# johndpope/SPEAK-hack

Measured on NVIDIA B200. Metric: irfd_train_pairs_per_sec_256, higher is better.
Workload: dtype bf16

## Files before the change

include/irfd_b200.h:

```cpp
#ifndef IRFD_B200_H_
#define IRFD_B200_H_

#include <stddef.h>
#include <stdint.h>

#ifdef __cplusplus
extern "C" {
#endif

#define IRFD_ABI_VERSION 1

#define IRFD_OK 0
#define IRFD_ERR_INVALID_ARGUMENT (-1)
#define IRFD_ERR_CUDA (-2)

typedef struct CUstream_st* irfd_stream_t;

int irfd_abi_version(void);
const char* irfd_last_error(void);

int irfd_conv_gemm_m_tiles(int n, int h, int w);
int irfd_conv_gemm(const void* x, int n, int h, int w, int cin, const void* wk, int cout, int ksize, void* out,
                   void* out2, int mode, const float* bias, const float* nw, const float* noise, const float* sp1,
                   const float* s1, float* stat_sum, float* stat_sq, int force_block_n, irfd_stream_t stream);
// ... 36 lines not shown
                  void* out, long long rows, int c, int relu, int groups, irfd_stream_t stream);
long long irfd_bn_bwd_workspace_bytes(long long rows, int c, int groups);
int irfd_bn_backward(const void* g1, const void* g2, const void* act, const void* z, const float* mean,
                     const float* rstd, const float* gamma, const float* beta, void* dz, void* g_out, float* dgamma,
                     float* dbeta, float grad_beta, int batch_stats, long long rows, int c, int groups, void* workspace,
                     long long workspace_bytes, irfd_stream_t stream);

int irfd_bn_eval_affine_sets(const float* const* running_mean, const float* const* running_var,
                             const float* const* gamma, const float* const* beta, float eps, float* scale, float* shift,
                             int c, int nsets, irfd_stream_t stream);
int irfd_bn_finalize_sets(const float* psum, const float* psq, int tiles, int c, long long count, float eps,
                          float momentum, float* mean, float* rstd, float* const* running_mean,
                          float* const* running_var, int running_updates, int groups, int nsets,
                          irfd_stream_t stream);
int irfd_bn_apply_sets(const void* z, const float* mean, const float* rstd, const float* const* gamma,
                       const float* const* beta, const void* res, const float* mean2, const float* rstd2,
                       const float* const* gamma2, const float* const* beta2, void* out, void* mask_bits,
                       long long rows, int c, int relu, int groups, int nsets, irfd_stream_t stream);
int irfd_bn_backward_sets(const void* g1, const void* g2, const void* act, int act_is_bits, const void* z,
                          const float* mean, const float* rstd, const float* const* gamma, const float* const* beta,
                          void* dz, void* g_out, float* const* dgamma, float* const* dbeta, float grad_beta,
                          int batch_stats, long long rows, int c, int groups, int nsets, void* workspace,
                          long long workspace_bytes, irfd_stream_t stream);

int irfd_conv_gemm_bnbwd_grouped(const void* x, int n, int h, int w, int cin, const void* wk, int cout, int ksize,
                                 void* out, const void* bn_z, const float* bn_mean, const float* bn_rstd,
                                 const float* const* bn_gamma, const float* const* bn_beta, float* partial,
                                 int stat_groups, int wgroups, int force_block_n, irfd_stream_t stream);
int irfd_conv_gemm_bnbwd_res_grouped(const void* x, int n, int h, int w, int cin, const void* wk, int cout, int ksize,
                                     void* out, const void* bn_z, const float* bn_mean, const float* bn_rstd,
                                     const void* g2, const void* mask_bits, float* partial, int stat_groups,
                                     int wgroups, int force_block_n, irfd_stream_t stream);
int irfd_bn_backward_finish_sets(const void* g, const void* z, const float* mean, const float* rstd,
                                 const float* const* gamma, void* dz, float* const* dgamma, float* const* dbeta,
                                 float grad_beta, int batch_stats, long long rows, int c, int groups, int nsets,
                                 const float* partial, int tiles, void* workspace, long long workspace_bytes,
                                 irfd_stream_t stream);

int irfd_pack_conv_weight(const float* w, void* dst, int o, int i, int taps, int mode, int kpad, irfd_stream_t stream);
int irfd_im2col_stem(const float* x, void* col, int n, int h, int w, int kpad, irfd_stream_t stream);
int irfd_im2col_3x3s2(const void* a, void* col, int n, int h, int w, int c, irfd_stream_t stream);
int irfd_col2im_3x3s2(const void* dcol, void* dx, int n, int h, int w, int c, irfd_stream_t stream);
int irfd_subsample2(const void* a, void* out, int n, int h, int w, int c, irfd_stream_t stream);
int irfd_scatter_add_s2(const void* a, const void* b, void* out, int n, int h, int w, int c, irfd_stream_t stream);
int irfd_maxpool_fwd(const void* a, void* out, void* argmax, int n, int h, int w, int c, irfd_stream_t stream);
int irfd_maxpool_bwd(const void* dout, const void* dout2, const void* argmax, void* dx, int n, int h, int w, int c,
// ... 73 lines not shown
```

speak_hack_b200/csrc/bn.cu:

```cuda
#include "host_util.h"
#include "rowvec.cuh"

namespace irfd {

constexpr int kMaxGroups = 4;
constexpr int kMaxSets = 4;
struct FSet {
  const float* p[kMaxSets];
};
struct FSetM {
  float* p[kMaxSets];
};
constexpr int kFinCh = 8;
constexpr int kFinLanes = 64;
constexpr int kFinThreads = kFinCh * kFinLanes;
constexpr int kFinWarps = kFinThreads / 32;
constexpr int kFinBatch = 8;

__device__ __forceinline__ void fin_partial_sums(const float* __restrict__ p0, const float* __restrict__ p1, size_t stride0,
                                                 size_t stride1, int n, int lane, double& a, double& b) {
  a = 0.0;
  b = 0.0;
  for (int t = lane; t < n; t += kFinLanes * kFinBatch) {
    float x[kFinBatch], y[kFinBatch];
#pragma unroll
    for (int u = 0; u < kFinBatch; ++u) {
      const int tt = t + u * kFinLanes;
      x[u] = tt < n ? __ldg(p0 + (size_t)tt * stride0) : 0.f;
      y[u] = tt < n ? __ldg(p1 + (size_t)tt * stride1) : 0.f;
    }
#pragma unroll
    for (int u = 0; u < kFinBatch; ++u) {
      a += (double)x[u];
      b += (double)y[u];
    }
  }
}

__device__ __forceinline__ void fin_block_sums(double& a, double& b, double (*sa)[kFinCh], double (*sb)[kFinCh]) {
#pragma unroll
  for (int o = kFinCh; o < 32; o <<= 1) {
    a += __shfl_xor_sync(0xffffffffu, a, o);
    b += __shfl_xor_sync(0xffffffffu, b, o);
  }
  const int w = threadIdx.x >> 5, l = threadIdx.x & 31;
  __syncthreads();
  if (l < kFinCh) {
    sa[w][l] = a;
    sb[w][l] = b;
  }
  __syncthreads();
  if (threadIdx.x < kFinCh) {
    a = 0.0;
    b = 0.0;
#pragma unroll 8
    for (int i = 0; i < kFinWarps; ++i) {
      a += sa[i][threadIdx.x];
      b += sb[i][threadIdx.x];
    }
  }
}

__global__ void __launch_bounds__(kFinThreads, 2)
bn_finalize_kernel(const float* __restrict__ psum, const float* __restrict__ psq, int tiles, int C, double count,
                   float eps, float momentum, float* __restrict__ mean, float* __restrict__ rstd, FSetM running_mean_s,
                   FSetM running_var_s, int running_updates, int groups) {
  __shared__ double s_sum[kFinWarps][kFinCh];
  __shared__ double s_sq[kFinWarps][kFinCh];
  const int cl = threadIdx.x & (kFinCh - 1);
  const int lane = threadIdx.x / kFinCh;
  const int c = blockIdx.x * kFinCh + cl;
  psum += (size_t)blockIdx.y * groups * tiles * C;
  psq += (size_t)blockIdx.y * groups * tiles * C;
  mean += (size_t)blockIdx.y * groups * C;
  rstd += (size_t)blockIdx.y * groups * C;
  float* running_mean = running_mean_s.p[blockIdx.y];
  float* running_var = running_var_s.p[blockIdx.y];
  double gm[kMaxGroups], gv[kMaxGroups];
#pragma unroll
  for (int g = 0; g < kMaxGroups; ++g) {
    if (g < groups) {
      double a, b;
      fin_partial_sums(psum + (size_t)g * tiles * C + c, psq + (size_t)g * tiles * C + c, C, C, tiles, lane, a, b);
      fin_block_sums(a, b, s_sum, s_sq);
      if (threadIdx.x < kFinCh) {
        const double m = a / count;
        double var = b / count - m * m;
        if (var < 0.0) var = 0.0;
        mean[(size_t)g * C + c] = (float)m;
        rstd[(size_t)g * C + c] = (float)(1.0 / sqrt(var + (double)eps));
        gm[g] = m;
        gv[g] = count > 1.0 ? var * count / (count - 1.0) : var;
      }
    }
  }
  if (threadIdx.x < kFinCh && running_mean != nullptr) {
    float rm = running_mean[c], rv = running_var[c];
    for (int u = 0; u < running_updates; ++u)
#pragma unroll
      for (int i = 0; i < kMaxGroups; ++i) {
        if (i < groups) {
          const int g = (u & 1) ? groups - 1 - i : i;
          double mg = gm[0], vg = gv[0];
#pragma unroll
          for (int k = 1; k < kMaxGroups; ++k)
            if (k == g) {
              mg = gm[k];
              vg = gv[k];
            }
          rm = (1.f - momentum) * rm + momentum * (float)mg;
          rv = (1.f - momentum) * rv + momentum * (float)vg;
        }
      }
    running_mean[c] = rm;
    running_var[c] = rv;
  }
}

__global__ void bn_running_update_kernel(const float* __restrict__ mean, const float* __restrict__ rstd, float eps,
                                         double count, float momentum, float* __restrict__ running_mean,
                                         float* __restrict__ running_var, int C) {
  const int c = blockIdx.x * blockDim.x + threadIdx.x;
  if (c >= C) return;
  const double r = (double)rstd[c];
  double var = 1.0 / (r * r) - (double)eps;
  if (var < 0.0) var = 0.0;
  const double unbiased = count > 1.0 ? var * count / (count - 1.0) : var;
  running_mean[c] = (1.f - momentum) * running_mean[c] + momentum * mean[c];
  running_var[c] = (1.f - momentum) * running_var[c] + momentum * (float)unbiased;
}

__global__ void bn_eval_affine_kernel(const float* __restrict__ running_mean, const float* __restrict__ running_var,
                                      const float* __restrict__ gamma, const float* __restrict__ beta, float eps,
                                      float* __restrict__ scale, float* __restrict__ shift, int C) {
  const int c = blockIdx.x * blockDim.x + threadIdx.x;
// ... 130 lines not shown
                                                   const float (&m)[8], const float (&rs)[8], const float (&ga)[8],
                                                   const float (&be)[8], float (&g)[8]) {
  unpack8(qg, g);
  if (HAS_G2) {
    float h[8];
    unpack8(qh, h);
#pragma unroll
    for (int t = 0; t < 8; ++t) g[t] += h[t];
  }
  if (MASK == 1) {
    float a[8];
    unpack8(qa, a);
#pragma unroll
    for (int t = 0; t < 8; ++t) g[t] = a[t] > 0.f ? g[t] : 0.f;
  } else if (MASK == 2) {
#pragma unroll
    for (int t = 0; t < 8; ++t) g[t] = (ga[t] * ((zz[t] - m[t]) * rs[t]) + be[t]) > 0.f ? g[t] : 0.f;
  } else if (MASK == 3) {
#pragma unroll
    for (int t = 0; t < 8; ++t) g[t] = ((qa.x >> t) & 1u) ? g[t] : 0.f;
  }
}

template <bool HAS_G2, int MASK, bool G_OUT>
__global__ void __launch_bounds__(kRvThreads, 2)
bn_bwd_reduce_kernel(const __nv_bfloat16* __restrict__ g1, const __nv_bfloat16* __restrict__ g2,
                     const __nv_bfloat16* __restrict__ act, const __nv_bfloat16* __restrict__ z,
                     const float* __restrict__ mean, const float* __restrict__ rstd, FSet gamma_s, FSet beta_s,
                     float* __restrict__ partial, __nv_bfloat16* __restrict__ g_out, long long rows, int C,
                     int rows_per_blk, int gps, int reverse) {
  constexpr int RB = kRowBatch;
  const unsigned bx = reverse ? gridDim.x - 1 - blockIdx.x : blockIdx.x;
  const unsigned by = reverse ? gridDim.y - 1 - blockIdx.y : blockIdx.y;
  const float* __restrict__ gamma = gamma_s.p[by / gps];
  const float* __restrict__ beta = beta_s.p[by / gps];
  extern __shared__ float red_smem[];
  RowVec rv(C);
  {
    const size_t goff = (size_t)by * rows * C;
    g1 += goff;
    if (HAS_G2) g2 += goff;
    if (MASK == 1) act += goff;
    if (MASK == 3) act = reinterpret_cast<const __nv_bfloat16*>(reinterpret_cast<const uint8_t*>(act) + (goff >> 3));
    z += goff;
    if (G_OUT) g_out += goff;
    mean += (size_t)by * C;
    rstd += (size_t)by * C;
    partial += (size_t)by * gridDim.x * 2 * C;
  }
  float acc[2][8];
#pragma unroll
  for (int t = 0; t < 8; ++t) acc[0][t] = acc[1][t] = 0.f;
  if (rv.active) {
// ... 19 lines not shown
          qz[u] = ldg16(z + off);
          if (MASK == 1) qa[u] = ldg16(act + off);
          if (MASK == 3) qa[u].x = __ldg(reinterpret_cast<const uint8_t*>(act) + (off >> 3));
        }
      }
#pragma unroll
      for (int u = 0; u < RB; ++u) {
        const long long rr = r + (long long)u * rv.rows_par;
        if (rr < r1) {
          float g[8], zz[8];
          unpack8(qz[u], zz);
          bn_bwd_masked_grad<HAS_G2, MASK>(qg[u], qh[u], qa[u], zz, m, rs, ga, be, g);
          if (G_OUT) store8(g_out + (size_t)rr * C + rv.cv * 8, g);
#pragma unroll
          for (int t = 0; t < 8; ++t) {
            acc[0][t] += g[t];
            acc[1][t] += g[t] * ((zz[t] - m[t]) * rs[t]);
          }
        }
      }
    }
  }
  block_reduce_rows<2>(rv, C, acc, red_smem, partial + (size_t)bx * 2 * C, (size_t)C);
}

__global__ void __launch_bounds__(kFinThreads, 2)
bn_bwd_finalize_kernel(const float* __restrict__ partial, int nblk, int C, double count, FSetM dgamma_s, FSetM dbeta_s,
                       float beta_acc, float* __restrict__ c1, float* __restrict__ c2, int batch_stats, int groups) {
  __shared__ double s0s[kFinWarps][kFinCh];
  __shared__ double s1s[kFinWarps][kFinCh];
  const int cl = threadIdx.x & (kFinCh - 1);
  const int lane = threadIdx.x / kFinCh;
  const int c = blockIdx.x * kFinCh + cl;
  partial += (size_t)blockIdx.y * groups * nblk * 2 * C;
  c1 += (size_t)blockIdx.y * groups * C;
  c2 += (size_t)blockIdx.y * groups * C;
  float* __restrict__ dgamma = dgamma_s.p[blockIdx.y];
  float* __restrict__ dbeta = dbeta_s.p[blockIdx.y];
  double tot0 = 0.0, tot1 = 0.0;
  for (int g = 0; g < groups; ++g) {
    const float* pg = partial + (size_t)g * nblk * 2 * C + c;
    double s0, s1;
    fin_partial_sums(pg, pg + C, (size_t)2 * C, (size_t)2 * C, nblk, lane, s0, s1);
    fin_block_sums(s0, s1, s0s, s1s);
    if (threadIdx.x < kFinCh) {
      c1[(size_t)g * C + c] = batch_stats ? (float)(s0 / count) : 0.f;
      c2[(size_t)g * C + c] = batch_stats ? (float)(s1 / count) : 0.f;
      tot0 += s0;
      tot1 += s1;
    }
  }
  if (threadIdx.x < kFinCh) {
    dbeta[c] = (beta_acc != 0.f ? beta_acc * dbeta[c] : 0.f) + (float)tot0;
    dgamma[c] = (beta_acc != 0.f ? beta_acc * dgamma[c] : 0.f) + (float)tot1;
  }
}

template <bool HAS_G2, int MASK, bool G_OUT>
__global__ void __launch_bounds__(kRvThreads, 2)
bn_bwd_apply_kernel(const __nv_bfloat16* __restrict__ g1, const __nv_bfloat16* __restrict__ g2,
                    const __nv_bfloat16* __restrict__ act, const __nv_bfloat16* __restrict__ z,
                    const float* __restrict__ mean, const float* __restrict__ rstd, FSet gamma_s, FSet beta_s,
                    const float* __restrict__ c1, const float* __restrict__ c2, __nv_bfloat16* __restrict__ dz,
                    __nv_bfloat16* __restrict__ g_out, long long rows, int C, int rows_per_blk, int gps) {
  constexpr int RB = kRowBatch;
  RowVec rv(C);
  if (!rv.active) return;
  const float* __restrict__ gamma = gamma_s.p[blockIdx.y / gps];
  const float* __restrict__ beta = beta_s.p[blockIdx.y / gps];
  {
    const size_t goff = (size_t)blockIdx.y * rows * C;
    g1 += goff;
    if (HAS_G2) g2 += goff;
    if (MASK == 1) act += goff;
    if (MASK == 3) act = reinterpret_cast<const __nv_bfloat16*>(reinterpret_cast<const uint8_t*>(act) + (goff >> 3));
    z += goff;
    dz += goff;
// ... 49 lines not shown
static int zigzag() {
  static int v = [] {
    const char* e = getenv("IRFD_ZIGZAG");
    return e ? atoi(e) : 1;
  }();
  return v;
}

struct BnBwdLaunch {
  dim3 grid;
  size_t smem;
  cudaStream_t stream;
  const __nv_bfloat16 *g1, *g2, *act, *z;
  const float *mean, *rstd;
  FSet gamma, beta;
  float *partial, *c1, *c2;
  __nv_bfloat16 *dz, *g_out;
  FSetM dgamma, dbeta;
  float grad_beta;
  int batch_stats;
  long long grows;
  int c, rpb, nblk, groups;
  int nsets, gps;
};

template <bool HAS_G2, int MASK>
static void launch_bn_bwd(const BnBwdLaunch& L) {
  prefer_max_shared_carveout(reinterpret_cast<const void*>(&bn_bwd_reduce_kernel<HAS_G2, MASK, true>));
  prefer_max_shared_carveout(reinterpret_cast<const void*>(&bn_bwd_reduce_kernel<HAS_G2, MASK, false>));
  prefer_max_shared_carveout(reinterpret_cast<const void*>(&bn_bwd_apply_kernel<HAS_G2, MASK, false>));
  prefer_max_shared_carveout(reinterpret_cast<const void*>(&bn_bwd_apply_kernel<false, 0, false>));
  prefer_max_shared_carveout(reinterpret_cast<const void*>(&bn_bwd_finalize_kernel));
  if (L.g_out != nullptr)
    bn_bwd_reduce_kernel<HAS_G2, MASK, true><<<L.grid, kRvThreads, L.smem, L.stream>>>(
        L.g1, L.g2, L.act, L.z, L.mean, L.rstd, L.gamma, L.beta, L.partial, L.g_out, L.grows, L.c, L.rpb, L.gps,
        zigzag());
  else
    bn_bwd_reduce_kernel<HAS_G2, MASK, false><<<L.grid, kRvThreads, L.smem, L.stream>>>(
        L.g1, L.g2, L.act, L.z, L.mean, L.rstd, L.gamma, L.beta, L.partial, nullptr, L.grows, L.c, L.rpb, L.gps,
        zigzag());
  bn_bwd_finalize_kernel<<<dim3(L.c / kFinCh, L.nsets), kFinThreads, 0, L.stream>>>(L.partial, L.nblk, L.c, (double)L.grows,
                                                                             L.dgamma, L.dbeta, L.grad_beta, L.c1, L.c2,
                                                                             L.batch_stats, L.gps);
  if (L.g_out != nullptr)
    bn_bwd_apply_kernel<false, 0, false><<<L.grid, kRvThreads, 0, L.stream>>>(
        L.g_out, nullptr, nullptr, L.z, L.mean, L.rstd, L.gamma, L.beta, L.c1, L.c2, L.dz, nullptr, L.grows, L.c, L.rpb,
        L.gps);
  else
    bn_bwd_apply_kernel<HAS_G2, MASK, false><<<L.grid, kRvThreads, 0, L.stream>>>(
        L.g1, L.g2, L.act, L.z, L.mean, L.rstd, L.gamma, L.beta, L.c1, L.c2, L.dz, nullptr, L.grows, L.c, L.rpb,
        L.gps);
}

}

using namespace irfd;

static FSet make_fset(const float* const* ptrs, int nsets) {
  FSet f;
  for (int i = 0; i < kMaxSets; ++i) f.p[i] = (ptrs != nullptr && i < nsets) ? ptrs[i] : nullptr;
  return f;
}
static FSetM make_fsetm(float* const* ptrs, int nsets) {
  FSetM f;
  for (int i = 0; i < kMaxSets; ++i) f.p[i] = (ptrs != nullptr && i < nsets) ? ptrs[i] : nullptr;
  return f;
}

extern "C" int irfd_bn_finalize_sets(const float* psum, const float* psq, int tiles, int c, long long count, float eps,
                                     float momentum, float* mean, float* rstd, float* const* running_mean,
                                     float* const* running_var, int running_updates, int groups, int nsets,
                                     cudaStream_t stream) {
  IRFD_CHECK_ARG(psum && psq && mean && rstd && tiles > 0 && c > 0 && count > 0, "bn_finalize: bad argument");
  IRFD_CHECK_ARG(groups >= 1 && groups <= kMaxGroups, "bn_finalize: 1..4 statistic groups per set");
  IRFD_CHECK_ARG(nsets >= 1 && nsets <= kMaxSets, "bn_finalize: 1..4 parameter sets");
  IRFD_CHECK_ARG(c % kFinCh == 0, "bn_finalize: C must be a multiple of 8 (got %d)", c);
  IRFD_CHECK_ARG((running_mean == nullptr) == (running_var == nullptr), "bn_finalize: running buffers come in pairs");
  bn_finalize_kernel<<<dim3(c / kFinCh, nsets), kFinThreads, 0, stream>>>(psum, psq, tiles, c, (double)count, eps, momentum,
                                                                     mean, rstd, make_fsetm(running_mean, nsets),
                                                                     make_fsetm(running_var, nsets), running_updates,
                                                                     groups);
  IRFD_CHECK_LAUNCH();
  return IRFD_OK;
}

extern "C" int irfd_bn_finalize(const float* psum, const float* psq, int tiles, int c, long long count, float eps,
                                float momentum, float* mean, float* rstd, float* running_mean, float* running_var,
                                int running_updates, int groups, cudaStream_t stream) {
  float* rm[1] = {running_mean};
  float* rv[1] = {running_var};
  return irfd_bn_finalize_sets(psum, psq, tiles, c, count, eps, momentum, mean, rstd, running_mean ? rm : nullptr,
                               running_var ? rv : nullptr, running_updates, groups, 1, stream);
}

extern "C" int irfd_bn_running_update(const float* mean, const float* rstd, float eps, long long count, float momentum,
                                      float* running_mean, float* running_var, int c, cudaStream_t stream) {
  IRFD_CHECK_ARG(mean && rstd && running_mean && running_var && c > 0 && count > 0, "bn_running_update: bad argument");
  bn_running_update_kernel<<<(c + 255) / 256, 256, 0, stream>>>(mean, rstd, eps, (double)count, momentum, running_mean,
                                                                 running_var, c);
  IRFD_CHECK_LAUNCH();
  return IRFD_OK;
}

extern "C" int irfd_bn_eval_affine(const float* running_mean, const float* running_var, const float* gamma,
// ... 53 lines not shown
  IRFD_CHECK_LAUNCH();
  return IRFD_OK;
}

extern "C" int irfd_bn_apply(const void* z, const float* mean, const float* rstd, const float* gamma, const float* beta,
                             const void* res, const float* mean2, const float* rstd2, const float* gamma2,
                             const float* beta2, void* out, long long rows, int c, int relu, int groups,
                             cudaStream_t stream) {
  const float* g1[1] = {gamma};
  const float* b1[1] = {beta};
  const float* g2[1] = {gamma2};
  const float* b2[1] = {beta2};
  return irfd_bn_apply_sets(z, mean, rstd, g1, b1, res, mean2, rstd2, g2, b2, out, nullptr, rows, c, relu, groups, 1,
                            stream);
}

extern "C" long long irfd_bn_bwd_workspace_bytes(long long rows, int c, int groups) {
  if (groups < 1) groups = 1;
  int nblk, rpb;
  plan_row_blocks(rows / groups, c, num_sms(), &nblk, &rpb);
  return (long long)(nblk * 2 + 2) * groups * c * 4;
}

extern "C" int irfd_bn_backward_sets(const void* g1, const void* g2, const void* act, int act_is_bits, const void* z,
                                     const float* mean, const float* rstd, const float* const* gamma,
                                     const float* const* beta, void* dz, void* g_out, float* const* dgamma,
                                     float* const* dbeta, float grad_beta, int batch_stats, long long rows, int c,
                                     int groups, int nsets, void* workspace, long long workspace_bytes,
                                     cudaStream_t stream) {
  IRFD_CHECK_ARG(g1 && z && mean && rstd && gamma && dz && dgamma && dbeta && workspace, "bn_backward: null pointer");
  IRFD_CHECK_ARG(c % 8 == 0 && c <= 2048 && rows > 0, "bn_backward: C must be a multiple of 8 and <= 2048");
  IRFD_CHECK_ARG(groups >= 1 && rows % groups == 0, "bn_backward: rows must split evenly into groups");
  IRFD_CHECK_ARG(nsets >= 1 && nsets <= kMaxSets && groups % nsets == 0,
                 "bn_backward: groups must split evenly into 1..4 sets");
  const long long grows = rows / groups;
  int nblk, rpb;
  plan_row_blocks(grows, c, num_sms(), &nblk, &rpb);
  IRFD_CHECK_ARG(workspace_bytes >= (long long)(nblk * 2 + 2) * groups * c * 4, "bn_backward: workspace too small");
  float* partial = reinterpret_cast<float*>(workspace);
  float* c1 = partial + (size_t)groups * nblk * 2 * c;
  float* c2 = c1 + (size_t)groups * c;
  int rows_par = kRvThreads / (c / 8);
  if (rows_par < 1) rows_par = 1;
  const size_t smem = (size_t)2 * rows_par * c * sizeof(float);
  auto G1 = reinterpret_cast<const __nv_bfloat16*>(g1);
  auto G2 = reinterpret_cast<const __nv_bfloat16*>(g2);
  auto A = reinterpret_cast<const __nv_bfloat16*>(act);
  auto Z = reinterpret_cast<const __nv_bfloat16*>(z);
  BnBwdLaunch L;
  L.grid = dim3(nblk, groups);
  L.smem = smem;
  L.stream = stream;
  L.g1 = G1; L.g2 = G2; L.act = A; L.z = Z;
  L.mean = mean; L.rstd = rstd;
  L.gamma = make_fset(gamma, nsets);
  L.beta = make_fset(beta, nsets);
  L.partial = partial; L.c1 = c1; L.c2 = c2;
  L.dz = reinterpret_cast<__nv_bfloat16*>(dz);
  L.g_out = reinterpret_cast<__nv_bfloat16*>(g_out);
  L.dgamma = make_fsetm(dgamma, nsets);
  L.dbeta = make_fsetm(dbeta, nsets);
  L.grad_beta = grad_beta; L.batch_stats = batch_stats;
  L.grows = grows; L.c = c; L.rpb = rpb; L.nblk = nblk; L.groups = groups;
  L.nsets = nsets; L.gps = groups / nsets;
  const bool has_beta = beta != nullptr && beta[0] != nullptr;
  const int mask = A != nullptr ? (act_is_bits ? 3 : 1) : (has_beta ? 2 : 0);
  if (G2 != nullptr) {
    if (mask == 0) launch_bn_bwd<true, 0>(L);
    else if (mask == 1) launch_bn_bwd<true, 1>(L);
    else if (mask == 2) launch_bn_bwd<true, 2>(L);
    else launch_bn_bwd<true, 3>(L);
  } else {
    if (mask == 0) launch_bn_bwd<false, 0>(L);
    else if (mask == 1) launch_bn_bwd<false, 1>(L);
    else if (mask == 2) launch_bn_bwd<false, 2>(L);
    else launch_bn_bwd<false, 3>(L);
  }
  IRFD_CHECK_LAUNCH();
  return IRFD_OK;
}

extern "C" int irfd_bn_backward_finish_sets(const void* g, const void* z, const float* mean, const float* rstd,
                                            const float* const* gamma, void* dz, float* const* dgamma,
                                            float* const* dbeta, float grad_beta, int batch_stats, long long rows,
                                            int c, int groups, int nsets, const float* partial, int tiles,
                                            void* workspace, long long workspace_bytes, cudaStream_t stream) {
  IRFD_CHECK_ARG(g && z && mean && rstd && gamma && dz && dgamma && dbeta && partial && workspace,
                 "bn_backward_finish: null pointer");
  IRFD_CHECK_ARG(c % 8 == 0 && c <= 2048 && rows > 0 && tiles > 0, "bn_backward_finish: bad shape");
  IRFD_CHECK_ARG(groups >= 1 && rows % groups == 0, "bn_backward_finish: rows must split evenly into groups");
  IRFD_CHECK_ARG(nsets >= 1 && nsets <= kMaxSets && groups % nsets == 0,
                 "bn_backward_finish: groups must split evenly into 1..4 sets");
  IRFD_CHECK_ARG(workspace_bytes >= (long long)2 * groups * c * 4, "bn_backward_finish: workspace too small");
  const long long grows = rows / groups;
  int nblk, rpb;
  plan_row_blocks(grows, c, num_sms(), &nblk, &rpb);
  float* c1 = reinterpret_cast<float*>(workspace);
  float* c2 = c1 + (size_t)groups * c;
  const FSet ga = make_fset(gamma, nsets);
  const FSet be = make_fset(nullptr, nsets);
  const int gps = groups / nsets;
  prefer_max_shared_carveout(reinterpret_cast<const void*>(&bn_bwd_apply_kernel<false, 0, false>));
  prefer_max_shared_carveout(reinterpret_cast<const void*>(&bn_bwd_finalize_kernel));
  bn_bwd_finalize_kernel<<<dim3(c / kFinCh, nsets), kFinThreads, 0, stream>>>(partial, tiles, c, (double)grows,
                                                                        make_fsetm(dgamma, nsets),
                                                                        make_fsetm(dbeta, nsets), grad_beta, c1, c2,
                                                                        batch_stats, gps);
  bn_bwd_apply_kernel<false, 0, false><<<dim3(nblk, groups), kRvThreads, 0, stream>>>(
      reinterpret_cast<const __nv_bfloat16*>(g), nullptr, nullptr, reinterpret_cast<const __nv_bfloat16*>(z), mean, rstd,
      ga, be, c1, c2, reinterpret_cast<__nv_bfloat16*>(dz), nullptr, grows, c, rpb, gps);
  IRFD_CHECK_LAUNCH();
  return IRFD_OK;
}

extern "C" int irfd_bn_backward(const void* g1, const void* g2, const void* act, const void* z, const float* mean,
                                const float* rstd, const float* gamma, const float* beta, void* dz, void* g_out,
                                float* dgamma, float* dbeta, float grad_beta, int batch_stats, long long rows, int c,
                                int groups, void* workspace, long long workspace_bytes, cudaStream_t stream) {
  const float* ga[1] = {gamma};
  const float* be[1] = {beta};
  float* dg[1] = {dgamma};
  float* db[1] = {dbeta};
  return irfd_bn_backward_sets(g1, g2, act, 0, z, mean, rstd, ga, be, dz, g_out, dg, db, grad_beta, batch_stats, rows,
                               c, groups, 1, workspace, workspace_bytes, stream);
}
```

speak_hack_b200/ops.py:

```python
from __future__ import annotations

import ctypes
import os
import weakref
from typing import Optional

import torch

from . import _lib

BF16 = torch.bfloat16
F32 = torch.float32

EPI_PLAIN, EPI_STATS, EPI_STYLE = 0, 1, 2
PACK_FPROP, PACK_DGRAD, PACK_DCOL, PACK_FLAT = 0, 1, 2, 3

launch_count = 0


def _stream() -> int:
    return torch.cuda.current_stream().cuda_stream


def _ptr(t: Optional[torch.Tensor]) -> Optional[int]:
# ... 502 lines not shown
def bn_apply_sets(z, mean, rstd, gammas, betas, res=None, bn2=None, relu=True, groups=1, want_mask=False):
    _chk(z, BF16, "z")
    c = z.shape[-1]
    rows = z.numel() // c
    out = torch.empty_like(z)
    bits = torch.empty((rows, c // 8), dtype=torch.uint8, device=z.device) if want_mask else None
    m2 = r2 = g2 = b2 = None
    if bn2 is not None:
        m2, r2, g2, b2 = bn2
    _call("irfd_bn_apply_sets", z.data_ptr(), mean.data_ptr(), rstd.data_ptr(), _ptr_array(gammas), _ptr_array(betas),
          _ptr(res), _ptr(m2), _ptr(r2), _ptr_array(g2) if g2 is not None else _ptr_array([None] * len(gammas)),
          _ptr_array(b2) if b2 is not None else _ptr_array([None] * len(gammas)), out.data_ptr(), _ptr(bits), rows, c,
          1 if relu else 0, groups, len(gammas), _stream())
    return (out, bits) if want_mask else out


def _bn_bwd_bytes(rows, c, has_g2, mask_units, want_g_out):
    n_in = 2 + (1 if has_g2 else 0) + mask_units
    if want_g_out:
        return 2.0 * rows * c * (n_in + 1 + 3)
    return 2.0 * rows * c * (2 * n_in + 1)


def bn_backward_sets(g1, g2, act, z, mean, rstd, gammas, betas=None, dgammas=None, dbetas=None, want_g_out=False,
                     batch_stats=True, groups=1, act_bits=None):
    lib = _lib.load()
    c = z.shape[-1]
    rows = z.numel() // c
    nsets = len(gammas)
    dz = torch.empty_like(z)
    g_out = torch.empty_like(z) if want_g_out else None
    if dgammas is None:
        dg_all = torch.empty((nsets, c), dtype=F32, device=z.device)
        db_all = torch.empty((nsets, c), dtype=F32, device=z.device)
        dgammas, dbetas = list(dg_all.unbind(0)), list(db_all.unbind(0))
    ws = workspace(lib.irfd_bn_bwd_workspace_bytes(rows, c, groups), z.device)
    if act_bits is not None and act is not None:
        raise _lib.IrfdError("bn_backward_sets: pass act or act_bits, not both")
    mask_units = 1.0 if act is not None else (1.0 / 16 if act_bits is not None else 0.0)
    nbytes = _bn_bwd_bytes(rows, c, g2 is not None, mask_units, want_g_out)
    with _timed("bn_backward (reduce+finalize+apply, HBM)", nbytes):
        _call("irfd_bn_backward_sets", g1.data_ptr(), _ptr(g2), _ptr(act if act_bits is None else act_bits),
              0 if act_bits is None else 1, z.data_ptr(), mean.data_ptr(),
              rstd.data_ptr(), _ptr_array(gammas), _ptr_array(betas) if betas is not None else None, dz.data_ptr(),
              _ptr(g_out), _ptr_array(dgammas), _ptr_array(dbetas), 0.0, 1 if batch_stats else 0, rows, c, groups, nsets,
              ws.data_ptr(), ws.numel(), _stream(), launches=3)
    if want_g_out:
        return dz, dgammas, dbetas, g_out
    return dz, dgammas, dbetas


def bn_backward_finish_sets(g, z, mean, rstd, gammas, partial, dgammas=None, dbetas=None, batch_stats=True, groups=1):
    c = z.shape[-1]
    rows = z.numel() // c
    nsets = len(gammas)
    dz = torch.empty_like(z)
    if dgammas is None:
        dg_all = torch.empty((nsets, c), dtype=F32, device=z.device)
        db_all = torch.empty((nsets, c), dtype=F32, device=z.device)
        dgammas, dbetas = list(dg_all.unbind(0)), list(db_all.unbind(0))
    if partial.shape[0] % groups:
        raise _lib.IrfdError("bn_backward_finish_sets: partial rows do not split into the statistic groups")
    ws = workspace(2 * groups * c * 4, z.device)
    with _timed("bn_backward (reduce+finalize+apply, HBM)", 2.0 * rows * c * 3):
        _call("irfd_bn_backward_finish_sets", g.data_ptr(), z.data_ptr(), mean.data_ptr(), rstd.data_ptr(),
              _ptr_array(gammas), dz.data_ptr(), _ptr_array(dgammas), _ptr_array(dbetas), 0.0, 1 if batch_stats else 0,
              rows, c, groups, nsets, partial.data_ptr(), partial.shape[0] // groups, ws.data_ptr(), ws.numel(), _stream(),
              launches=2)
    return dz, dgammas, dbetas
# ... 357 lines not shown
```

Before: 889.1.

## Fuse BN backward finalize into reduce via ticket tail; parallelize finalize over groups

Adds an optional fused BN-backward path in which the last reduce block per group, chosen by an atomic ticket, computes the per-channel sums, and the last group per set writes dgamma/dbeta. This removes the separate finalize launch. The finalize kernels are also templated so that several statistic groups are reduced concurrently within one block, using quad-level shuffles and shared-memory staging. The fused path relies on a Python-side ticket pool and threadfence ordering, and is only used when the caller passes fused=True.

```diff
diff --git a/include/irfd_b200.h b/include/irfd_b200.h
--- a/include/irfd_b200.h
+++ b/include/irfd_b200.h
@@ -82,6 +82,13 @@
                           void* dz, void* g_out, float* const* dgamma, float* const* dbeta, float grad_beta,
                           int batch_stats, long long rows, int c, int groups, int nsets, void* workspace,
                           long long workspace_bytes, irfd_stream_t stream);
+long long irfd_bn_bwd_fused_workspace_bytes(long long rows, int c, int groups);
+int irfd_bn_backward_sets_fused(const void* g1, const void* g2, const void* act, int act_is_bits, const void* z,
+                                const float* mean, const float* rstd, const float* const* gamma,
+                                const float* const* beta, void* dz, void* g_out, float* const* dgamma,
+                                float* const* dbeta, float grad_beta, int batch_stats, long long rows, int c, int groups,
+                                int nsets, void* workspace, long long workspace_bytes, unsigned int* tickets,
+                                irfd_stream_t stream);
 
 int irfd_conv_gemm_bnbwd_grouped(const void* x, int n, int h, int w, int cin, const void* wk, int cout, int ksize,
                                  void* out, const void* bn_z, const float* bn_mean, const float* bn_rstd,
diff --git a/speak_hack_b200/csrc/bn.cu b/speak_hack_b200/csrc/bn.cu
--- a/speak_hack_b200/csrc/bn.cu
+++ b/speak_hack_b200/csrc/bn.cu
@@ -14,7 +14,7 @@
 constexpr int kFinCh = 8;
 constexpr int kFinLanes = 64;
 constexpr int kFinThreads = kFinCh * kFinLanes;
-constexpr int kFinWarps = kFinThreads / 32;
+constexpr int kFinQuads = kFinLanes / 4;
 constexpr int kFinBatch = 8;
 
 __device__ __forceinline__ void fin_partial_sums(const float* __restrict__ p0, const float* __restrict__ p1, size_t stride0,
@@ -37,80 +37,89 @@
   }
 }
 
-__device__ __forceinline__ void fin_block_sums(double& a, double& b, double (*sa)[kFinCh], double (*sb)[kFinCh]) {
-#pragma unroll
-  for (int o = kFinCh; o < 32; o <<= 1) {
-    a += __shfl_xor_sync(0xffffffffu, a, o);
-    b += __shfl_xor_sync(0xffffffffu, b, o);
-  }
-  const int w = threadIdx.x >> 5, l = threadIdx.x & 31;
+template <int CH>
+__device__ __forceinline__ void fin_block_sums(double& a, double& b, int part, int lane, int cl, double* sa, double* sb) {
+  a += __shfl_xor_sync(0xffffffffu, a, CH);
+  b += __shfl_xor_sync(0xffffffffu, b, CH);
+  a += __shfl_xor_sync(0xffffffffu, a, 2 * CH);
+  b += __shfl_xor_sync(0xffffffffu, b, 2 * CH);
+  double* qa = sa + (size_t)part * kFinQuads * CH;
+  double* qb = sb + (size_t)part * kFinQuads * CH;
   __syncthreads();
-  if (l < kFinCh) {
-    sa[w][l] = a;
-    sb[w][l] = b;
+  if ((lane & 3) == 0) {
+    qa[(lane >> 2) * CH + cl] = a;
+    qb[(lane >> 2) * CH + cl] = b;
   }
   __syncthreads();
-  if (threadIdx.x < kFinCh) {
+  if (lane == 0) {
     a = 0.0;
     b = 0.0;
 #pragma unroll 8
-    for (int i = 0; i < kFinWarps; ++i) {
-      a += sa[i][threadIdx.x];
-      b += sb[i][threadIdx.x];
-    }
-  }
-}
-
+    for (int i = 0; i < kFinQuads; ++i) {
+      a += qa[i * CH + cl];
+      b += qb[i * CH + cl];
+    }
+  }
+}
+
+template <int CH, int GP>
+struct FinShape {
+  static_assert(CH * kFinLanes * GP == kFinThreads, "512 threads");
+  int part, lane, cl;
+  __device__ FinShape() {
+    const int t = threadIdx.x % (CH * kFinLanes);
+    part = threadIdx.x / (CH * kFinLanes);
+    lane = t / CH;
+    cl = t % CH;
+  }
+};
+
+template <int CH, int GP>
 __global__ void __launch_bounds__(kFinThreads, 2)
 bn_finalize_kernel(const float* __restrict__ psum, const float* __restrict__ psq, int tiles, int C, double count,
                    float eps, float momentum, float* __restrict__ mean, float* __restrict__ rstd, FSetM running_mean_s,
                    FSetM running_var_s, int running_updates, int groups) {
-  __shared__ double s_sum[kFinWarps][kFinCh];
-  __shared__ double s_sq[kFinWarps][kFinCh];
-  const int cl = threadIdx.x & (kFinCh - 1);
-  const int lane = threadIdx.x / kFinCh;
-  const int c = blockIdx.x * kFinCh + cl;
+  __shared__ double s_sum[GP * kFinQuads * CH];
+  __shared__ double s_sq[GP * kFinQuads * CH];
+  __shared__ double s_m[kMaxGroups][CH], s_v[kMaxGroups][CH];
+  const FinShape<CH, GP> sh;
+  const int c = blockIdx.x * CH + sh.cl;
   psum += (size_t)blockIdx.y * groups * tiles * C;
   psq += (size_t)blockIdx.y * groups * tiles * C;
   mean += (size_t)blockIdx.y * groups * C;
   rstd += (size_t)blockIdx.y * groups * C;
-  float* running_mean = running_mean_s.p[blockIdx.y];
-  float* running_var = running_var_s.p[blockIdx.y];
-  double gm[kMaxGroups], gv[kMaxGroups];
-#pragma unroll
-  for (int g = 0; g < kMaxGroups; ++g) {
-    if (g < groups) {
-      double a, b;
-      fin_partial_sums(psum + (size_t)g * tiles * C + c, psq + (size_t)g * tiles * C + c, C, C, tiles, lane, a, b);
-      fin_block_sums(a, b, s_sum, s_sq);
-      if (threadIdx.x < kFinCh) {
-        const double m = a / count;
-        double var = b / count - m * m;
-        if (var < 0.0) var = 0.0;
-        mean[(size_t)g * C + c] = (float)m;
-        rstd[(size_t)g * C + c] = (float)(1.0 / sqrt(var + (double)eps));
-        gm[g] = m;
-        gv[g] = count > 1.0 ? var * count / (count - 1.0) : var;
-      }
-    }
-  }
-  if (threadIdx.x < kFinCh && running_mean != nullptr) {
+  float* running_mean = running_mean_s.p[0];
+  float* running_var = running_var_s.p[0];
+#pragma unroll
+  for (int k = 1; k < kMaxSets; ++k)
+    if (k == (int)blockIdx.y) {
+      running_mean = running_mean_s.p[k];
+      running_var = running_var_s.p[k];
+    }
+  for (int g0 = 0; g0 < groups; g0 += GP) {
+    const int g = g0 + sh.part;
+    const int gg = g < groups ? g : groups - 1;
+    double a, b;
+    fin_partial_sums(psum + (size_t)gg * tiles * C + c, psq + (size_t)gg * tiles * C + c, C, C, tiles, sh.lane, a, b);
+    fin_block_sums<CH>(a, b, sh.part, sh.lane, sh.cl, s_sum, s_sq);
+    if (sh.lane == 0 && g < groups) {
+      const double m = a / count;
+      double var = b / count - m * m;
+      if (var < 0.0) var = 0.0;
+      mean[(size_t)g * C + c] = (float)m;
+      rstd[(size_t)g * C + c] = (float)(1.0 / sqrt(var + (double)eps));
+      s_m[g][sh.cl] = m;
+      s_v[g][sh.cl] = count > 1.0 ? var * count / (count - 1.0) : var;
+    }
+  }
+  __syncthreads();
+  if (threadIdx.x < CH && running_mean != nullptr) {
     float rm = running_mean[c], rv = running_var[c];
     for (int u = 0; u < running_updates; ++u)
-#pragma unroll
-      for (int i = 0; i < kMaxGroups; ++i) {
-        if (i < groups) {
-          const int g = (u & 1) ? groups - 1 - i : i;
-          double mg = gm[0], vg = gv[0];
-#pragma unroll
-          for (int k = 1; k < kMaxGroups; ++k)
-            if (k == g) {
-              mg = gm[k];
-              vg = gv[k];
-            }
-          rm = (1.f - momentum) * rm + momentum * (float)mg;
-          rv = (1.f - momentum) * rv + momentum * (float)vg;
-        }
+      for (int i = 0; i < groups; ++i) {
+        const int g = (u & 1) ? groups - 1 - i : i;
+        rm = (1.f - momentum) * rm + momentum * (float)s_m[g][sh.cl];
+        rv = (1.f - momentum) * rv + momentum * (float)s_v[g][sh.cl];
       }
     running_mean[c] = rm;
     running_var[c] = rv;
@@ -287,13 +296,90 @@
   }
 }
 
-template <bool HAS_G2, int MASK, bool G_OUT>
+struct FinTail {
+  unsigned* tickets;
+  double* dsum;
+  float *c1, *c2;
+  FSetM dgamma, dbeta;
+  float beta_acc;
+  int batch_stats;
+};
+constexpr int kTailQuads = 16;
+constexpr int kTailWarpLanes = kRvThreads / kTailQuads;
+constexpr size_t kTailSmem = 2 * kTailWarpLanes * 4 * kTailQuads * sizeof(double);
+
+template <class Emit>
+__device__ __forceinline__ void fin_tail_sums(const float* p0, const float* p1, size_t stride, int n, int C, double* sw,
+                                              Emit emit) {
+  const int q = threadIdx.x / kTailQuads;
+  const int cq = threadIdx.x % kTailQuads;
+  constexpr int CH = 4 * kTailQuads;
+  for (int cb = 0; cb < C; cb += CH) {
+    const int c = cb + cq * 4;
+    double a[4][4], b[4][4];
+#pragma unroll
+    for (int j = 0; j < 4; ++j)
+#pragma unroll
+      for (int t = 0; t < 4; ++t) a[j][t] = b[j][t] = 0.0;
+    if (c < C) {
+      for (int r0 = 4 * q; r0 < n; r0 += kFinLanes) {
+        float4 x[4], y[4];
+#pragma unroll
+        for (int j = 0; j < 4; ++j)
+          if (r0 + j < n) {
+            x[j] = __ldcg(reinterpret_cast<const float4*>(p0 + (size_t)(r0 + j) * stride + c));
+            y[j] = __ldcg(reinterpret_cast<const float4*>(p1 + (size_t)(r0 + j) * stride + c));
+          }
+#pragma unroll
+        for (int j = 0; j < 4; ++j)
+          if (r0 + j < n) {
+            a[j][0] += (double)x[j].x; a[j][1] += (double)x[j].y; a[j][2] += (double)x[j].z; a[j][3] += (double)x[j].w;
+            b[j][0] += (double)y[j].x; b[j][1] += (double)y[j].y; b[j][2] += (double)y[j].z; b[j][3] += (double)y[j].w;
+          }
+      }
+    }
+    __syncthreads();
+#pragma unroll
+    for (int t = 0; t < 4; ++t) {
+      sw[q * CH + cq * 4 + t] = (a[0][t] + a[1][t]) + (a[2][t] + a[3][t]);
+      sw[(kTailWarpLanes + q) * CH + cq * 4 + t] = (b[0][t] + b[1][t]) + (b[2][t] + b[3][t]);
+    }
+    __syncthreads();
+    if (threadIdx.x < CH && cb + (int)threadIdx.x < C) {
+      double s0 = 0.0, s1 = 0.0;
+#pragma unroll
+      for (int i = 0; i < kTailWarpLanes; ++i) {
+        s0 += sw[i * CH + threadIdx.x];
+        s1 += sw[(kTailWarpLanes + i) * CH + threadIdx.x];
+      }
+      emit(cb + (int)threadIdx.x, s0, s1);
+    }
+  }
+}
+
+__device__ __forceinline__ bool fin_take_ticket(unsigned* ticket, unsigned total) {
+  __shared__ unsigned s_last;
+  __threadfence();
+  __syncthreads();
+  if (threadIdx.x == 0) {
+    const unsigned t = atomicAdd(ticket, 1u);
+    s_last = t == total - 1;
+    if (t == total - 1) {
+      *ticket = 0u;
+      __threadfence();
+    }
+  }
+  __syncthreads();
+  return s_last;
+}
+
+template <bool HAS_G2, int MASK, bool G_OUT, bool TAIL>
 __global__ void __launch_bounds__(kRvThreads, 2)
 bn_bwd_reduce_kernel(const __nv_bfloat16* __restrict__ g1, const __nv_bfloat16* __restrict__ g2,
                      const __nv_bfloat16* __restrict__ act, const __nv_bfloat16* __restrict__ z,
                      const float* __restrict__ mean, const float* __restrict__ rstd, FSet gamma_s, FSet beta_s,
                      float* __restrict__ partial, __nv_bfloat16* __restrict__ g_out, long long rows, int C,
-                     int rows_per_blk, int gps, int reverse) {
+                     int rows_per_blk, int gps, int reverse, FinTail tail) {
   constexpr int RB = kRowBatch;
   const unsigned bx = reverse ? gridDim.x - 1 - blockIdx.x : blockIdx.x;
   const unsigned by = reverse ? gridDim.y - 1 - blockIdx.y : blockIdx.y;
@@ -359,37 +445,96 @@
     }
   }
   block_reduce_rows<2>(rv, C, acc, red_smem, partial + (size_t)bx * 2 * C, (size_t)C);
-}
-
+  if constexpr (!TAIL) return;
+  if (!fin_take_ticket(tail.tickets + by, gridDim.x)) return;
+  const double count = (double)rows;
+  fin_tail_sums(partial, partial + C, (size_t)2 * C, gridDim.x, C, reinterpret_cast<double*>(red_smem),
+                [&](int c, double s0, double s1) {
+                  tail.c1[(size_t)by * C + c] = tail.batch_stats ? (float)(s0 / count) : 0.f;
+                  tail.c2[(size_t)by * C + c] = tail.batch_stats ? (float)(s1 / count) : 0.f;
+                  tail.dsum[((size_t)by * 2) * C + c] = s0;
+                  tail.dsum[((size_t)by * 2 + 1) * C + c] = s1;
+                });
+  const int set = by / gps;
+  if (!fin_take_ticket(tail.tickets + gridDim.y + set, gps)) return;
+  float* __restrict__ dgamma = tail.dgamma.p[0];
+  float* __restrict__ dbeta = tail.dbeta.p[0];
+#pragma unroll
+  for (int k = 1; k < kMaxSets; ++k)
+    if (k == set) {
+      dgamma = tail.dgamma.p[k];
+      dbeta = tail.dbeta.p[k];
+    }
+  for (int c = threadIdx.x; c < C; c += kRvThreads) {
+    double tot0 = 0.0, tot1 = 0.0;
+    for (int g = set * gps; g < (set + 1) * gps; ++g) {
+      tot0 += __ldcg(tail.dsum + ((size_t)g * 2) * C + c);
+      tot1 += __ldcg(tail.dsum + ((size_t)g * 2 + 1) * C + c);
+    }
+    dbeta[c] = (tail.beta_acc != 0.f ? tail.beta_acc * dbeta[c] : 0.f) + (float)tot0;
+    dgamma[c] = (tail.beta_acc != 0.f ? tail.beta_acc * dgamma[c] : 0.f) + (float)tot1;
+  }
+}
+
+template <int CH, int GP>
 __global__ void __launch_bounds__(kFinThreads, 2)
 bn_bwd_finalize_kernel(const float* __restrict__ partial, int nblk, int C, double count, FSetM dgamma_s, FSetM dbeta_s,
                        float beta_acc, float* __restrict__ c1, float* __restrict__ c2, int batch_stats, int groups) {
-  __shared__ double s0s[kFinWarps][kFinCh];
-  __shared__ double s1s[kFinWarps][kFinCh];
-  const int cl = threadIdx.x & (kFinCh - 1);
-  const int lane = threadIdx.x / kFinCh;
-  const int c = blockIdx.x * kFinCh + cl;
+  __shared__ double s0s[GP * kFinQuads * CH];
+  __shared__ double s1s[GP * kFinQuads * CH];
+  __shared__ double s_t0[kMaxGroups][CH], s_t1[kMaxGroups][CH];
+  const FinShape<CH, GP> sh;
+  const int c = blockIdx.x * CH + sh.cl;
   partial += (size_t)blockIdx.y * groups * nblk * 2 * C;
   c1 += (size_t)blockIdx.y * groups * C;
   c2 += (size_t)blockIdx.y * groups * C;
-  float* __restrict__ dgamma = dgamma_s.p[blockIdx.y];
-  float* __restrict__ dbeta = dbeta_s.p[blockIdx.y];
-  double tot0 = 0.0, tot1 = 0.0;
-  for (int g = 0; g < groups; ++g) {
-    const float* pg = partial + (size_t)g * nblk * 2 * C + c;
+  float* __restrict__ dgamma = dgamma_s.p[0];
+  float* __restrict__ dbeta = dbeta_s.p[0];
+#pragma unroll
+  for (int k = 1; k < kMaxSets; ++k)
+    if (k == (int)blockIdx.y) {
+      dgamma = dgamma_s.p[k];
+      dbeta = dbeta_s.p[k];
+    }
+  for (int g0 = 0; g0 < groups; g0 += GP) {
+    const int g = g0 + sh.part;
+    const int gg = g < groups ? g : groups - 1;
+    const float* pg = partial + (size_t)gg * nblk * 2 * C + c;
     double s0, s1;
-    fin_partial_sums(pg, pg + C, (size_t)2 * C, (size_t)2 * C, nblk, lane, s0, s1);
-    fin_block_sums(s0, s1, s0s, s1s);
-    if (threadIdx.x < kFinCh) {
+    fin_partial_sums(pg, pg + C, (size_t)2 * C, (size_t)2 * C, nblk, sh.lane, s0, s1);
+    fin_block_sums<CH>(s0, s1, sh.part, sh.lane, sh.cl, s0s, s1s);
+    if (sh.lane == 0 && g < groups) {
       c1[(size_t)g * C + c] = batch_stats ? (float)(s0 / count) : 0.f;
       c2[(size_t)g * C + c] = batch_stats ? (float)(s1 / count) : 0.f;
-      tot0 += s0;
-      tot1 += s1;
-    }
-  }
-  if (threadIdx.x < kFinCh) {
+      s_t0[g][sh.cl] = s0;
+      s_t1[g][sh.cl] = s1;
+    }
+  }
+  __syncthreads();
+  if (threadIdx.x < CH) {
+    double tot0 = 0.0, tot1 = 0.0;
+    for (int g = 0; g < groups; ++g) {
+      tot0 += s_t0[g][sh.cl];
+      tot1 += s_t1[g][sh.cl];
+    }
     dbeta[c] = (beta_acc != 0.f ? beta_acc * dbeta[c] : 0.f) + (float)tot0;
     dgamma[c] = (beta_acc != 0.f ? beta_acc * dgamma[c] : 0.f) + (float)tot1;
+  }
+}
+
+static inline bool fin_pairs(int gps) { return gps >= 2; }
+
+static void launch_bn_bwd_finalize(const float* partial, int nblk, int C, double count, FSetM dgamma, FSetM dbeta,
+                                   float beta_acc, float* c1, float* c2, int batch_stats, int gps, int nsets,
+                                   cudaStream_t stream) {
+  if (fin_pairs(gps)) {
+    prefer_max_shared_carveout(reinterpret_cast<const void*>(&bn_bwd_finalize_kernel<4, 2>));
+    bn_bwd_finalize_kernel<4, 2><<<dim3(C / 4, nsets), kFinThreads, 0, stream>>>(partial, nblk, C, count, dgamma, dbeta,
+                                                                                 beta_acc, c1, c2, batch_stats, gps);
+  } else {
+    prefer_max_shared_carveout(reinterpret_cast<const void*>(&bn_bwd_finalize_kernel<8, 1>));
+    bn_bwd_finalize_kernel<8, 1><<<dim3(C / 8, nsets), kFinThreads, 0, stream>>>(partial, nblk, C, count, dgamma, dbeta,
+                                                                                 beta_acc, c1, c2, batch_stats, gps);
   }
 }
 
@@ -485,26 +630,38 @@
   long long grows;
   int c, rpb, nblk, groups;
   int nsets, gps;
+  FinTail tail;
 };
 
 template <bool HAS_G2, int MASK>
 static void launch_bn_bwd(const BnBwdLaunch& L) {
-  prefer_max_shared_carveout(reinterpret_cast<const void*>(&bn_bwd_reduce_kernel<HAS_G2, MASK, true>));
-  prefer_max_shared_carveout(reinterpret_cast<const void*>(&bn_bwd_reduce_kernel<HAS_G2, MASK, false>));
+  prefer_max_shared_carveout(reinterpret_cast<const void*>(&bn_bwd_reduce_kernel<HAS_G2, MASK, true, false>));
+  prefer_max_shared_carveout(reinterpret_cast<const void*>(&bn_bwd_reduce_kernel<HAS_G2, MASK, false, false>));
   prefer_max_shared_carveout(reinterpret_cast<const void*>(&bn_bwd_apply_kernel<HAS_G2, MASK, false>));
   prefer_max_shared_carveout(reinterpret_cast<const void*>(&bn_bwd_apply_kernel<false, 0, false>));
-  prefer_max_shared_carveout(reinterpret_cast<const void*>(&bn_bwd_finalize_kernel));
-  if (L.g_out != nullptr)
-    bn_bwd_reduce_kernel<HAS_G2, MASK, true><<<L.grid, kRvThreads, L.smem, L.stream>>>(
+  if (L.tail.tickets != nullptr) {
+    prefer_max_shared_carveout(reinterpret_cast<const void*>(&bn_bwd_reduce_kernel<HAS_G2, MASK, true, true>));
+    prefer_max_shared_carveout(reinterpret_cast<const void*>(&bn_bwd_reduce_kernel<HAS_G2, MASK, false, true>));
+  }
+  if (L.g_out != nullptr && L.tail.tickets != nullptr)
+    bn_bwd_reduce_kernel<HAS_G2, MASK, true, true><<<L.grid, kRvThreads, L.smem, L.stream>>>(
         L.g1, L.g2, L.act, L.z, L.mean, L.rstd, L.gamma, L.beta, L.partial, L.g_out, L.grows, L.c, L.rpb, L.gps,
-        zigzag());
+        zigzag(), L.tail);
+  else if (L.g_out != nullptr)
+    bn_bwd_reduce_kernel<HAS_G2, MASK, true, false><<<L.grid, kRvThreads, L.smem, L.stream>>>(
+        L.g1, L.g2, L.act, L.z, L.mean, L.rstd, L.gamma, L.beta, L.partial, L.g_out, L.grows, L.c, L.rpb, L.gps,
+        zigzag(), L.tail);
+  else if (L.tail.tickets != nullptr)
+    bn_bwd_reduce_kernel<HAS_G2, MASK, false, true><<<L.grid, kRvThreads, L.smem, L.stream>>>(
+        L.g1, L.g2, L.act, L.z, L.mean, L.rstd, L.gamma, L.beta, L.partial, nullptr, L.grows, L.c, L.rpb, L.gps,
+        zigzag(), L.tail);
   else
-    bn_bwd_reduce_kernel<HAS_G2, MASK, false><<<L.grid, kRvThreads, L.smem, L.stream>>>(
+    bn_bwd_reduce_kernel<HAS_G2, MASK, false, false><<<L.grid, kRvThreads, L.smem, L.stream>>>(
         L.g1, L.g2, L.act, L.z, L.mean, L.rstd, L.gamma, L.beta, L.partial, nullptr, L.grows, L.c, L.rpb, L.gps,
-        zigzag());
-  bn_bwd_finalize_kernel<<<dim3(L.c / kFinCh, L.nsets), kFinThreads, 0, L.stream>>>(L.partial, L.nblk, L.c, (double)L.grows,
-                                                                             L.dgamma, L.dbeta, L.grad_beta, L.c1, L.c2,
-                                                                             L.batch_stats, L.gps);
+        zigzag(), L.tail);
+  if (L.tail.tickets == nullptr)
+    launch_bn_bwd_finalize(L.partial, L.nblk, L.c, (double)L.grows, L.dgamma, L.dbeta, L.grad_beta, L.c1, L.c2,
+                           L.batch_stats, L.gps, L.nsets, L.stream);
   if (L.g_out != nullptr)
     bn_bwd_apply_kernel<false, 0, false><<<L.grid, kRvThreads, 0, L.stream>>>(
         L.g_out, nullptr, nullptr, L.z, L.mean, L.rstd, L.gamma, L.beta, L.c1, L.c2, L.dz, nullptr, L.grows, L.c, L.rpb,
@@ -539,10 +696,14 @@
   IRFD_CHECK_ARG(nsets >= 1 && nsets <= kMaxSets, "bn_finalize: 1..4 parameter sets");
   IRFD_CHECK_ARG(c % kFinCh == 0, "bn_finalize: C must be a multiple of 8 (got %d)", c);
   IRFD_CHECK_ARG((running_mean == nullptr) == (running_var == nullptr), "bn_finalize: running buffers come in pairs");
-  bn_finalize_kernel<<<dim3(c / kFinCh, nsets), kFinThreads, 0, stream>>>(psum, psq, tiles, c, (double)count, eps, momentum,
-                                                                     mean, rstd, make_fsetm(running_mean, nsets),
-                                                                     make_fsetm(running_var, nsets), running_updates,
-                                                                     groups);
+  if (fin_pairs(groups))
+    bn_finalize_kernel<4, 2><<<dim3(c / 4, nsets), kFinThreads, 0, stream>>>(
+        psum, psq, tiles, c, (double)count, eps, momentum, mean, rstd, make_fsetm(running_mean, nsets),
+        make_fsetm(running_var, nsets), running_updates, groups);
+  else
+    bn_finalize_kernel<8, 1><<<dim3(c / 8, nsets), kFinThreads, 0, stream>>>(
+        psum, psq, tiles, c, (double)count, eps, momentum, mean, rstd, make_fsetm(running_mean, nsets),
+        make_fsetm(running_var, nsets), running_updates, groups);
   IRFD_CHECK_LAUNCH();
   return IRFD_OK;
 }
@@ -642,12 +803,17 @@
   return (long long)(nblk * 2 + 2) * groups * c * 4;
 }
 
-extern "C" int irfd_bn_backward_sets(const void* g1, const void* g2, const void* act, int act_is_bits, const void* z,
-                                     const float* mean, const float* rstd, const float* const* gamma,
-                                     const float* const* beta, void* dz, void* g_out, float* const* dgamma,
-                                     float* const* dbeta, float grad_beta, int batch_stats, long long rows, int c,
-                                     int groups, int nsets, void* workspace, long long workspace_bytes,
-                                     cudaStream_t stream) {
+extern "C" long long irfd_bn_bwd_fused_workspace_bytes(long long rows, int c, int groups) {
+  if (groups < 1) groups = 1;
+  return irfd_bn_bwd_workspace_bytes(rows, c, groups) + (long long)2 * groups * c * 8;
+}
+
+static int bn_backward_sets_impl(const void* g1, const void* g2, const void* act, int act_is_bits, const void* z,
+                                 const float* mean, const float* rstd, const float* const* gamma,
+                                 const float* const* beta, void* dz, void* g_out, float* const* dgamma,
+                                 float* const* dbeta, float grad_beta, int batch_stats, long long rows, int c,
+                                 int groups, int nsets, void* workspace, long long workspace_bytes, unsigned* tickets,
+                                 cudaStream_t stream) {
   IRFD_CHECK_ARG(g1 && z && mean && rstd && gamma && dz && dgamma && dbeta && workspace, "bn_backward: null pointer");
   IRFD_CHECK_ARG(c % 8 == 0 && c <= 2048 && rows > 0, "bn_backward: C must be a multiple of 8 and <= 2048");
   IRFD_CHECK_ARG(groups >= 1 && rows % groups == 0, "bn_backward: rows must split evenly into groups");
@@ -656,13 +822,15 @@
   const long long grows = rows / groups;
   int nblk, rpb;
   plan_row_blocks(grows, c, num_sms(), &nblk, &rpb);
-  IRFD_CHECK_ARG(workspace_bytes >= (long long)(nblk * 2 + 2) * groups * c * 4, "bn_backward: workspace too small");
+  const long long ws_need = (long long)(nblk * 2 + 2) * groups * c * 4 + (tickets ? (long long)2 * groups * c * 8 : 0);
+  IRFD_CHECK_ARG(workspace_bytes >= ws_need, "bn_backward: workspace too small");
   float* partial = reinterpret_cast<float*>(workspace);
   float* c1 = partial + (size_t)groups * nblk * 2 * c;
   float* c2 = c1 + (size_t)groups * c;
   int rows_par = kRvThreads / (c / 8);
   if (rows_par < 1) rows_par = 1;
-  const size_t smem = (size_t)2 * rows_par * c * sizeof(float);
+  size_t smem = (size_t)2 * rows_par * c * sizeof(float);
+  if (tickets != nullptr && smem < kTailSmem) smem = kTailSmem;
   auto G1 = reinterpret_cast<const __nv_bfloat16*>(g1);
   auto G2 = reinterpret_cast<const __nv_bfloat16*>(g2);
   auto A = reinterpret_cast<const __nv_bfloat16*>(act);
@@ -683,6 +851,11 @@
   L.grad_beta = grad_beta; L.batch_stats = batch_stats;
   L.grows = grows; L.c = c; L.rpb = rpb; L.nblk = nblk; L.groups = groups;
   L.nsets = nsets; L.gps = groups / nsets;
+  L.tail.tickets = tickets;
+  L.tail.dsum = reinterpret_cast<double*>(c2 + (size_t)groups * c);
+  L.tail.c1 = c1; L.tail.c2 = c2;
+  L.tail.dgamma = L.dgamma; L.tail.dbeta = L.dbeta;
+  L.tail.beta_acc = grad_beta; L.tail.batch_stats = batch_stats;
   const bool has_beta = beta != nullptr && beta[0] != nullptr;
   const int mask = A != nullptr ? (act_is_bits ? 3 : 1) : (has_beta ? 2 : 0);
   if (G2 != nullptr) {
@@ -698,6 +871,29 @@
   }
   IRFD_CHECK_LAUNCH();
   return IRFD_OK;
+}
+
+extern "C" int irfd_bn_backward_sets(const void* g1, const void* g2, const void* act, int act_is_bits, const void* z,
+                                     const float* mean, const float* rstd, const float* const* gamma,
+                                     const float* const* beta, void* dz, void* g_out, float* const* dgamma,
+                                     float* const* dbeta, float grad_beta, int batch_stats, long long rows, int c,
+                                     int groups, int nsets, void* workspace, long long workspace_bytes,
+                                     cudaStream_t stream) {
+  return bn_backward_sets_impl(g1, g2, act, act_is_bits, z, mean, rstd, gamma, beta, dz, g_out, dgamma, dbeta,
+                               grad_beta, batch_stats, rows, c, groups, nsets, workspace, workspace_bytes, nullptr,
+                               stream);
+}
+
+extern "C" int irfd_bn_backward_sets_fused(const void* g1, const void* g2, const void* act, int act_is_bits,
+                                           const void* z, const float* mean, const float* rstd,
+                                           const float* const* gamma, const float* const* beta, void* dz, void* g_out,
+                                           float* const* dgamma, float* const* dbeta, float grad_beta, int batch_stats,
+                                           long long rows, int c, int groups, int nsets, void* workspace,
+                                           long long workspace_bytes, unsigned int* tickets, cudaStream_t stream) {
+  IRFD_CHECK_ARG(tickets != nullptr, "bn_backward_fused: null ticket array");
+  return bn_backward_sets_impl(g1, g2, act, act_is_bits, z, mean, rstd, gamma, beta, dz, g_out, dgamma, dbeta,
+                               grad_beta, batch_stats, rows, c, groups, nsets, workspace, workspace_bytes, tickets,
+                               stream);
 }
 
 extern "C" int irfd_bn_backward_finish_sets(const void* g, const void* z, const float* mean, const float* rstd,
@@ -721,11 +917,8 @@
   const FSet be = make_fset(nullptr, nsets);
   const int gps = groups / nsets;
   prefer_max_shared_carveout(reinterpret_cast<const void*>(&bn_bwd_apply_kernel<false, 0, false>));
-  prefer_max_shared_carveout(reinterpret_cast<const void*>(&bn_bwd_finalize_kernel));
-  bn_bwd_finalize_kernel<<<dim3(c / kFinCh, nsets), kFinThreads, 0, stream>>>(partial, tiles, c, (double)grows,
-                                                                        make_fsetm(dgamma, nsets),
-                                                                        make_fsetm(dbeta, nsets), grad_beta, c1, c2,
-                                                                        batch_stats, gps);
+  launch_bn_bwd_finalize(partial, tiles, c, (double)grows, make_fsetm(dgamma, nsets), make_fsetm(dbeta, nsets),
+                         grad_beta, c1, c2, batch_stats, gps, nsets, stream);
   bn_bwd_apply_kernel<false, 0, false><<<dim3(nblk, groups), kRvThreads, 0, stream>>>(
       reinterpret_cast<const __nv_bfloat16*>(g), nullptr, nullptr, reinterpret_cast<const __nv_bfloat16*>(z), mean, rstd,
       ga, be, c1, c2, reinterpret_cast<__nv_bfloat16*>(dz), nullptr, grows, c, rpb, gps);
diff --git a/speak_hack_b200/ops.py b/speak_hack_b200/ops.py
--- a/speak_hack_b200/ops.py
+++ b/speak_hack_b200/ops.py
@@ -548,8 +548,24 @@
     return 2.0 * rows * c * (2 * n_in + 1)
 
 
+_TICKET_SLOTS = 1 << 16
+_tickets = {}
+
+
+def fin_tickets(n: int, device) -> int:
+    key = (device.type, device.index)
+    ent = _tickets.get(key)
+    if ent is None:
+        ent = _tickets[key] = [torch.zeros(_TICKET_SLOTS, dtype=torch.int32, device=device), 0]
+    pool, cur = ent
+    if cur + n > _TICKET_SLOTS:
+        cur = 0
+    ent[1] = cur + n
+    return pool.data_ptr() + 4 * cur
+
+
 def bn_backward_sets(g1, g2, act, z, mean, rstd, gammas, betas=None, dgammas=None, dbetas=None, want_g_out=False,
-                     batch_stats=True, groups=1, act_bits=None):
+                     batch_stats=True, groups=1, act_bits=None, fused=False):
     lib = _lib.load()
     c = z.shape[-1]
     rows = z.numel() // c
@@ -560,17 +576,23 @@
         dg_all = torch.empty((nsets, c), dtype=F32, device=z.device)
         db_all = torch.empty((nsets, c), dtype=F32, device=z.device)
         dgammas, dbetas = list(dg_all.unbind(0)), list(db_all.unbind(0))
-    ws = workspace(lib.irfd_bn_bwd_workspace_bytes(rows, c, groups), z.device)
+    if fused:
+        ws = workspace(lib.irfd_bn_bwd_fused_workspace_bytes(rows, c, groups), z.device)
+    else:
+        ws = workspace(lib.irfd_bn_bwd_workspace_bytes(rows, c, groups), z.device)
     if act_bits is not None and act is not None:
         raise _lib.IrfdError("bn_backward_sets: pass act or act_bits, not both")
     mask_units = 1.0 if act is not None else (1.0 / 16 if act_bits is not None else 0.0)
     nbytes = _bn_bwd_bytes(rows, c, g2 is not None, mask_units, want_g_out)
+    args = (g1.data_ptr(), _ptr(g2), _ptr(act if act_bits is None else act_bits), 0 if act_bits is None else 1,
+            z.data_ptr(), mean.data_ptr(), rstd.data_ptr(), _ptr_array(gammas),
+            _ptr_array(betas) if betas is not None else None, dz.data_ptr(), _ptr(g_out), _ptr_array(dgammas),
+            _ptr_array(dbetas), 0.0, 1 if batch_stats else 0, rows, c, groups, nsets, ws.data_ptr(), ws.numel())
     with _timed("bn_backward (reduce+finalize+apply, HBM)", nbytes):
-        _call("irfd_bn_backward_sets", g1.data_ptr(), _ptr(g2), _ptr(act if act_bits is None else act_bits),
-              0 if act_bits is None else 1, z.data_ptr(), mean.data_ptr(),
-              rstd.data_ptr(), _ptr_array(gammas), _ptr_array(betas) if betas is not None else None, dz.data_ptr(),
-              _ptr(g_out), _ptr_array(dgammas), _ptr_array(dbetas), 0.0, 1 if batch_stats else 0, rows, c, groups, nsets,
-              ws.data_ptr(), ws.numel(), _stream(), launches=3)
+        if fused:
+            _call("irfd_bn_backward_sets_fused", *args, fin_tickets(groups + nsets, z.device), _stream(), launches=2)
+        else:
+            _call("irfd_bn_backward_sets", *args, _stream(), launches=3)
     if want_g_out:
         return dz, dgammas, dbetas, g_out
     return dz, dgammas, dbetas
```

Measured after the change: 899.5 (median of 6 runs). +1.2%, better.
